# Jutho/KrylovKit.jl

Measured on NVIDIA H100. Metric: eigsolve_lanczos_operator_applications_per_sec, higher is better.
Workload: dtype f64

## Files before the change

krylovkit.jl_b200/csrc/basis.cu:

```cuda
#include "tsk.cuh"
#include <cmath>
#include <algorithm>

int32_t b2k_enqueue_dot(b2k_ctx* ctx, const void* q, void* x, int64_t n, const void* qprev,
                        int sprev_slot, int slot, int accum_slot);
int32_t b2k_enqueue_axpy_dev(b2k_ctx* ctx, void* x, const void* q, int s_slot, int64_t n);
int32_t b2k_enqueue_apply(b2k_ctx* ctx, const b2k_op* op, const VecRef& x, const VecRef& y,
                          double a0, double a1, bool shifted, const VecRef* dotv, int dot_slot);

using namespace tsk;

namespace {


template <typename T, bool UPDATE, bool PROJECT>
__global__ void __launch_bounds__(NTHREADS, 1)
k_phase(const __grid_constant__ PhaseParams<T> p, const __grid_constant__ ColList cl) {
    extern __shared__ __align__(128) uint8_t smem[];
    SmemView sm(smem);
    const int64_t ntiles = (p.n + Cfg<T>::R - 1) / Cfg<T>::R;
    const bool ragged = (p.n % Cfg<T>::R) != 0 && ((ntiles - 1) % gridDim.x) == blockIdx.x;
    pipe_setup(sm, ragged);
    Pipe st;
    if (threadIdx.x >= NCONS) producer_phase<T>(p, cl, sm, st);
    else consumer_phase<T, UPDATE, PROJECT>(p, sm, st);
}

template <typename T>
struct FusedParams {
    PhaseParams<T> ph[3];
    int32_t kind[3];
    int32_t nph;
    unsigned* barrier;
    unsigned barrier_base;
    const int* stop;
    FinalizeParams fin;
    PeerStep ps;
    unsigned long long* trace;
};

template <typename T>
__device__ __forceinline__ void peer_boundary(const FusedParams<T>& fp, int i, uint8_t* smem) {
    __threadfence();
    asm volatile("fence.proxy.async;" ::: "memory");
    __syncthreads();
    int* flag = reinterpret_cast<int*>(smem + OFF_RED + 256);
    if (threadIdx.x == 0) {
        const unsigned old = atomicAdd(fp.barrier, 1u);
        *flag = (old == fp.barrier_base + (unsigned)(i + 1) * gridDim.x - 1u);
    }
    __syncthreads();
    const PeerDev& pd = fp.ps.pd;
    const int tid = threadIdx.x;
    if (fp.ph[i].part_h == nullptr) {
        const unsigned long long sq = fp.ps.seq_norm;
        if (*flag && tid < 32) {
            __threadfence();
            double a = (tid < 16) ? partial_lane_sum(fp.ph[i].part_n, gridDim.x, 1, tid, 16) : 0.0;
            for (int o = 8; o > 0; o >>= 1) a += __shfl_xor_sync(0xffffffffu, a, o);
            if (tid == 0) peer_publish1(pd, PEER_CH_NORM, sq, a);
        }
        peer_wait(pd, PEER_CH_NORM, sq, tid);
        __syncthreads();
        return;
    }
    const unsigned long long seq = fp.ps.seq_coef[i];
    if (*flag && tid < NCONS) {
        __threadfence();
        const int k = fp.ph[i].k;
        const int L = coef_lanes(k);
        const int j = tid / L, l = tid % L;
        const bool valid = j < k;
        const double a = coef_colsum(fp.ph[i].part_h, gridDim.x, B2K_KSTRIDE, j, l, L, valid);
        if (valid && l == 0)
            for (int p = 0; p < pd.nranks; ++p) peer_slot(pd, p, PEER_CH_COEF, seq, pd.rank)[j] = a;
        __threadfence_system();
        named_bar_sync(1, NCONS);
        if (tid < pd.nranks) st_release_sys_u64(peer_flag(pd, tid, PEER_CH_COEF, seq, pd.rank), seq);
    }
    peer_wait(pd, PEER_CH_COEF, seq, tid);
    __syncthreads();
}

template <typename T>
__global__ void __launch_bounds__(NTHREADS, 1)
k_gs_fused(const __grid_constant__ FusedParams<T> fp, const __grid_constant__ ColList cl) {
    extern __shared__ __align__(128) uint8_t smem[];
    if (fp.stop && *reinterpret_cast<const volatile int*>(fp.stop)) {
        if (threadIdx.x == 0 && fp.nph > 1) atomicAdd(fp.barrier, (unsigned)(fp.nph - 1));
        return;
    }
    SmemView sm(smem);
    const bool tr0 = fp.trace && blockIdx.x == 0 && threadIdx.x == 0;
    if (tr0) b2k_trace(fp.trace, 10);
    const int64_t n = fp.ph[0].n;
    const int64_t ntiles = (n + Cfg<T>::R - 1) / Cfg<T>::R;
    const bool ragged = (n % Cfg<T>::R) != 0 && ((ntiles - 1) % gridDim.x) == blockIdx.x;
    pipe_setup(sm, ragged);
    Pipe st;
    const bool prod = threadIdx.x >= NCONS;
    if (fp.ps.on && fp.ps.seq_alpha && !prod) {
        peer_wait(fp.ps.pd, PEER_CH_ALPHA, fp.ps.seq_alpha, threadIdx.x);
        named_bar_sync(1, NCONS);
    }
    if (tr0) b2k_trace(fp.trace, 11);
    for (int i = 0; i < fp.nph; ++i) {
        if (prod) {
            producer_phase<T>(fp.ph[i], cl, sm, st);
        } else {
            if (fp.kind[i] == 0) consumer_phase<T, false, true>(fp.ph[i], sm, st);
            else if (fp.kind[i] == 1) consumer_phase<T, true, true>(fp.ph[i], sm, st);
            else consumer_phase<T, true, false>(fp.ph[i], sm, st);
        }
        if (tr0) b2k_trace(fp.trace, 12 + i);
        if (i + 1 < fp.nph) {
            if (fp.ps.on) peer_boundary<T>(fp, i, smem);
            else grid_barrier(fp.barrier, fp.barrier_base + (unsigned)(i + 1) * gridDim.x);
            if (tr0) b2k_trace(fp.trace, 15 + i);
        }
    }
    if (fp.fin.enabled && !prod) {
        double* sh = reinterpret_cast<double*>(smem + OFF_RED);
        int* flag = reinterpret_cast<int*>(smem + OFF_RED + 256);
        if (fp.ps.on) __threadfence_system();
        else __threadfence();
        named_bar_sync(1, NCONS);
        if (threadIdx.x == 0) {
            const unsigned t = atomicInc(fp.fin.ticket, gridDim.x - 1);
            *flag = (t == gridDim.x - 1);
        }
        named_bar_sync(1, NCONS);
        if (*flag) {
            __threadfence();
            if (fp.trace && threadIdx.x == 0) b2k_trace(fp.trace, 18);
            finalize_block(fp.fin, threadIdx.x, sh, fp.ps.on ? &fp.ps : nullptr);
            if (fp.trace && threadIdx.x == 0) b2k_trace(fp.trace, 19);
        }
    }
}

__global__ void __launch_bounds__(NCONS)
k_finalize(const double* __restrict__ A, const double* __restrict__ B, const double* __restrict__ N, int G,
           int stride, int k, double* __restrict__ res, int off, int noff) {
    __shared__ double sh[2];
    FinalizeParams f;
    f.A = A; f.B = B; f.N = N; f.G = G; f.stride = stride; f.k = k; f.res = res; f.off = off; f.noff = noff;
    f.rec = nullptr; f.alpha_col = -1; f.tol = 0.0; f.stop = nullptr; f.ticket = nullptr; f.enabled = 1;
    f.peer = 0; f.G_local = G; f.norm_done = 0;
    finalize_block(f, threadIdx.x, sh);
}

__global__ void k_lanczos_seed(double* rec, double beta, int* stop) {
    rec[2] = beta;
    rec[3] = 1.0 / beta;
    rec[4] = beta * beta;
    *stop = 0;
}

template <typename T>
__global__ void k_res_to_vec(const double* __restrict__ res, T* __restrict__ out, int k,
                             T alpha) {
    const int j = blockIdx.x * blockDim.x + threadIdx.x;
    if (j < k) out[j] = alpha * (T)res[j];
}

struct TransformParams {
    void* base;
    int64_t ld, n;
    int32_t m, keep, ldu;
    const double* U;
    int32_t u_in_smem;
};

constexpr int TR_OFF_U = NS * SLOT_BYTES;
constexpr int TR_U_BYTES = 232448 - TR_OFF_U - 256;
constexpr int TR_OFF_BAR = TR_OFF_U + TR_U_BYTES;
constexpr int TR_SMEM = TR_OFF_BAR + 2 * NS * 8;
constexpr int TJ = 36;
constexpr int TR_THREADS = NCONS + 32;

template <typename T, bool USM>
__global__ void __launch_bounds__(TR_THREADS, 1)
k_transform(const __grid_constant__ TransformParams p, const __grid_constant__ ColList cl) {
    using CF = Cfg<T>;
    using V16 = typename CF::V16;
    constexpr int R = CF::R, C = CF::C, VEC = CF::VEC;
    extern __shared__ __align__(128) uint8_t smem[];
    const uint32_t ring = smem_u32(smem);
    const uint32_t full = smem_u32(smem + TR_OFF_BAR), empty = full + NS * 8;
    T* Us = reinterpret_cast<T*>(smem + TR_OFF_U);
    const int pitch = ((p.keep + VEC - 1) / VEC) * VEC;
    if (threadIdx.x == 0) {
        for (int i = 0; i < NS; ++i) {
            mbar_init(full + 8 * i, 1);
            mbar_init(empty + 8 * i, NCONS / 32);
        }
        fence_mbar_init();
// ... 1391 lines not shown
    }

    B2K_TRY(b2k_enqueue_apply(ctx, op, rv, rw, 0.0, 1.0, false, nullptr, -1));
    B2K_TRY(b2k_vec_axpby(ctx, w, cols[k - 1], -beta_old, 1.0));
    B2K_TRY(b2k_enqueue_dot(ctx, rv.ptr, rw.ptr, pn.n, nullptr, -1, S_A0, -1));
    B2K_TRY(b2k_allreduce(ctx, ctx->d_res + S_A0, 1, pn.sharded));
    B2K_TRY(b2k_enqueue_axpy_dev(ctx, rw.ptr, rv.ptr, S_A0, pn.n));
    double alpha = 0.0, beta = 0.0;
    if (alg == B2K_MGS) {
        B2K_TRY(b2k_enqueue_dot(ctx, nullptr, rw.ptr, pn.n, nullptr, -1, S_N, -1));
        B2K_TRY(b2k_allreduce(ctx, ctx->d_res + S_N, 1, pn.sharded));
        B2K_TRY(b2k_fetch_results(ctx, S_A0 + 1, 0));
        alpha = ctx->h_res[S_A0];
        beta = sqrt(ctx->h_res[S_N]);
    } else if (alg == B2K_MGS2B) {
        if (fused_ok(ctx, K1, pn.sharded, ctx->dtype)) {
            if (f64) B2K_TRY(cgs_fused_t<double>(ctx, pn, rw, K1, 1, g_use_coop));
            else B2K_TRY(cgs_fused_t<float>(ctx, pn, rw, K1, 1, g_use_coop));
        } else {
            if (f64) B2K_TRY(cgs_pass_unfused_t<double>(ctx, pn, rw, K1, S_H, S_N));
            else B2K_TRY(cgs_pass_unfused_t<float>(ctx, pn, rw, K1, S_H, S_N));
        }
        B2K_TRY(b2k_fetch_results(ctx, S_A0 + 1, 0));
        alpha = ctx->h_res[S_A0] + ctx->h_res[S_H + k];
        beta = sqrt(ctx->h_res[S_N]);
    } else if (alg == B2K_MGS2) {
        B2K_TRY(mgs_sweep(ctx, pn, rw, K1, S_H, -1));
        B2K_TRY(b2k_enqueue_dot(ctx, nullptr, rw.ptr, pn.n, nullptr, -1, S_N, -1));
        B2K_TRY(b2k_allreduce(ctx, ctx->d_res + S_N, 1, pn.sharded));
        B2K_TRY(b2k_fetch_results(ctx, S_A0 + 1, 0));
        alpha = ctx->h_res[S_A0] + ctx->h_res[S_H + k];
        beta = sqrt(ctx->h_res[S_N]);
    } else {
        B2K_TRY(b2k_enqueue_dot(ctx, nullptr, rw.ptr, pn.n, nullptr, -1, S_N, -1));
        B2K_TRY(b2k_allreduce(ctx, ctx->d_res + S_N, 1, pn.sharded));
        B2K_TRY(b2k_fetch_results(ctx, S_A0 + 1, 0));
        alpha = ctx->h_res[S_A0];
        beta = sqrt(ctx->h_res[S_N]);
        double nold = sqrt(beta * beta + alpha * alpha + beta_old * beta_old);
        while (eps < beta && beta < eta * nold) {
            nold = beta;
            B2K_TRY(mgs_sweep(ctx, pn, rw, K1, S_H, -1));
            B2K_TRY(b2k_enqueue_dot(ctx, nullptr, rw.ptr, pn.n, nullptr, -1, S_N, -1));
            B2K_TRY(b2k_allreduce(ctx, ctx->d_res + S_N, 1, pn.sharded));
            B2K_TRY(b2k_fetch_results(ctx, S_N + 1, 0));
            alpha += ctx->h_res[S_H + k];
            beta = sqrt(ctx->h_res[S_N]);
        }
    }
    *alpha_out = alpha;
    *beta_out = beta;
    return B2K_OK;
}

bool g_use_chain = true;

bool chain_ok(const b2k_ctx* ctx, const b2k_op* op, const b2k_vec* cols, int32_t k, int32_t nsteps, int32_t alg,
              double beta_old) {
    if (!g_use_chain || !g_use_coop || (alg != B2K_CGS2 && alg != B2K_MGS2B) || nsteps < 1 || nsteps > B2K_MAX_CHAIN)
        return false;
    int64_t op_rows = 0, op_cols = 0;
    int32_t op_kind = -1;
    if (b2k_op_info(op, &op_rows, &op_cols, nullptr, &op_kind) != B2K_OK) return false;
    if ((op_kind != 0 && op_kind != 2) || beta_old == 0.0 || !(beta_old == beta_old)) return false;
    const int32_t sp = B2K_VEC_SPACE(cols[k]);
    if (sp < 0 || sp >= (int32_t)ctx->spaces.size()) return false;
    const B2kSpace& s = ctx->spaces[sp];
    if (ctx->nranks > 1) {
        if (!s.sharded || !b2k_peer_ok(ctx) || !b2k_op_has_peer_halo(op) || op_rows != s.n) return false;
    } else if (op_rows != s.n || op_cols != s.n) {
        return false;
    }
    const int C = ctx->dtype == B2K_F64 ? 8 : 16;
    const int K1 = k + nsteps;
    return (K1 + C - 1) / C <= NS && K1 <= MAXCH * C && K1 <= PEER_SLOT;
}

template <typename T>
int32_t chain_step_gs(b2k_ctx* ctx, const Panel& pn, int K1, const VecRef& rw, const VecRef& vprev,
                      const VecRef& rv, double* rec_prev, double* rec, double tol, const PeerStep* psp,
                      bool scale_after) {
    const int grid = grid_for_rows<T>(ctx, pn.n);
    ColList cl;
    for (int i = 0; i < K1; ++i) cl.c[i] = pn.idx[i];
    double* PA = b2k_part_set(ctx, 0);
    double* PN = b2k_part_set(ctx, 2);
    FusedParams<T> fp;
    memset(&fp, 0, sizeof(fp));
    PhaseParams<T> a = base_params<T>(pn, K1, rw.ptr, rw.ptr);
    a.nvec = 3; a.e1 = (const T*)vprev.ptr; a.e2 = (const T*)rv.ptr; a.store_x = 1;
    a.c1_dev = rec_prev + 2;
    a.c2_dev = rec + 0;
    a.part_h = PA;
    PhaseParams<T> c = base_params<T>(pn, K1, rw.ptr, rw.ptr);
    c.store_x = 1; c.coef = PA; c.coef_sets = grid; c.coef_stride = B2K_KSTRIDE;
    c.alphac = (T)-1; c.part_n = PN;
    fp.ph[0] = a; fp.kind[0] = 0; fp.ph[1] = c; fp.kind[1] = 2; fp.nph = 2;
    if (scale_after) {
        PhaseParams<T> sc = base_params<T>(pn, 0, rw.ptr, rw.ptr);
        sc.store_x = 1; sc.beta_mode = 2; sc.scale_mode = 1;
        sc.scale_norm = PN; sc.scale_G = grid; sc.scale_stride = 1; sc.scale_tol = tol;
        fp.ph[2] = sc; fp.kind[2] = 2; fp.nph = 3;
    }
    fp.stop = reinterpret_cast<const int*>(ctx->d_sync + B2K_SYNC_STOP);
    fp.trace = ctx->d_trace;
    fp.fin.A = PA; fp.fin.B = nullptr; fp.fin.N = PN; fp.fin.G = grid; fp.fin.stride = B2K_KSTRIDE;
    fp.fin.k = K1; fp.fin.res = nullptr; fp.fin.off = 0; fp.fin.noff = 0; fp.fin.rec = rec;
    fp.fin.alpha_col = K1 - 1; fp.fin.tol = tol;
    fp.fin.stop = reinterpret_cast<int*>(ctx->d_sync + B2K_SYNC_STOP);
    fp.fin.ticket = ctx->d_sync + B2K_SYNC_GSFIN; fp.fin.enabled = 1;
    fp.fin.peer = 0; fp.fin.G_local = grid; fp.fin.norm_done = 0;
    if (psp && psp->on) {
        const PeerStep& ps = *psp;
        fp.ps = ps;
        char* win = b2k_peer_local(ctx);
        auto slot = [&](int ch, unsigned long long seq) {
            return reinterpret_cast<double*>(win + PEER_OFF_SLOTS) + (size_t)((ch * 2 + (int)(seq & 1ull)) * PEER_MAXR) * PEER_SLOT;
        };
        fp.ph[0].c2_dev = slot(PEER_CH_ALPHA, ps.seq_alpha);
        fp.ph[0].c2_sets = ps.pd.nranks;
        fp.ph[0].c2_stride = PEER_SLOT;
        fp.ph[1].coef = slot(PEER_CH_COEF, ps.seq_coef[0]);
        fp.ph[1].coef_sets = ps.pd.nranks;
        fp.ph[1].coef_stride = PEER_SLOT;
        fp.fin.A = fp.ph[1].coef; fp.fin.G = ps.pd.nranks; fp.fin.stride = PEER_SLOT; fp.fin.peer = 1;
        const int last = fp.nph - 1;
        if (scale_after) {
            fp.ph[2].scale_norm = slot(PEER_CH_NORM, ps.seq_norm);
            fp.ph[2].scale_G = ps.pd.nranks;
            fp.ph[2].scale_stride = PEER_SLOT;
            fp.fin.norm_done = 1;
        }
        if (ps.seq_halo) {
            fp.ph[last].send_lo = ps.send_lo;
            fp.ph[last].send_hi = ps.send_hi;
            fp.ph[last].halo_dn = ps.send_lo ? reinterpret_cast<T*>(ps.pd.win[ps.pd.rank - 1] + ps.dn_off) : nullptr;
            fp.ph[last].halo_up = ps.send_hi ? reinterpret_cast<T*>(ps.pd.win[ps.pd.rank + 1] + ps.up_off) : nullptr;
        }
    }
    const int pr = b2k_prof_begin(ctx, 1, (2.0 * K1 + 3.0) * sizeof(T) * (double)pn.n);
    B2K_TRY(launch_fused<T>(ctx, fp, cl, grid));
    b2k_prof_end(ctx, pr);
    return B2K_OK;
}

int32_t lanczos_chain(b2k_ctx* ctx, const b2k_op* op, b2k_vec* cols, int32_t k, int32_t nsteps,
                      double beta_old, double tol, int32_t alg, double* alphas_out, double* betas_out,
                      int32_t* steps_done, b2k_vec* r_out) {
    const bool f64 = ctx->dtype == B2K_F64;
    const int32_t space = B2K_VEC_SPACE(cols[k]);
    double* rec0 = ctx->d_steps;
    int* d_stop = reinterpret_cast<int*>(ctx->d_sync + B2K_SYNC_STOP);
    {
        VecRef t;
        for (int i = 0; i <= k; ++i) B2K_TRY(b2k_resolve(ctx, cols[i], &t));
    }
    k_lanczos_seed<<<1, 1, 0, ctx->stream>>>(rec0, beta_old, d_stop);
    B2K_LAUNCH_CHECK(ctx);
    const bool inplace = g_chain_mode == 1;
    std::vector<b2k_vec> touched, Vh, Wh;
    touched.push_back(cols[k]);
    int32_t enq = 0, rc = B2K_OK;
    const bool dist = ctx->nranks > 1;
    unsigned long long halo_seq = 0;
    if (inplace) B2K_TRY(b2k_vec_scale(ctx, cols[k], cols[k], 1.0 / beta_old));
    for (int32_t i = 0; i < nsteps; ++i) {
        const int32_t K = k + i;
        const b2k_vec R = cols[K];
        b2k_vec V = R, W = -1;
        if (!inplace) {
            rc = b2k_vec_alloc(ctx, space, &V);
            if (rc != B2K_OK) break;
            touched.push_back(V);
        }
        rc = b2k_vec_alloc(ctx, space, &W);
        if (rc != B2K_OK) break;
        touched.push_back(W);
        VecRef rR, rV, rW, vprev;
        rc = b2k_resolve(ctx, R, &rR);
        if (rc == B2K_OK) rc = b2k_resolve(ctx, V, &rV);
        if (rc == B2K_OK) rc = b2k_resolve(ctx, W, &rW);
        if (rc == B2K_OK) rc = b2k_resolve(ctx, cols[K - 1], &vprev);
        if (rc != B2K_OK) break;
        double* rec_prev = rec0 + (size_t)B2K_REC * i;
        double* rec = rec0 + (size_t)B2K_REC * (i + 1);
        const bool scale_after = inplace && (i + 1 < nsteps);
        SpmvFuse fz;
        memset(&fz, 0, sizeof(fz));
        if (!inplace) {
            fz.xscale = rec_prev + 3;
            fz.vout = rV.ptr;
        }
        fz.stop = d_stop;
        fz.dot_self = 1;
        fz.l2_hints = g_l2_hints ? 1 : 0;
        fz.trace = ctx->d_trace;
        if (alg == B2K_MGS2B) {
            fz.dot_sub_vec = vprev.ptr;
            fz.dot_sub_scale = rec_prev + 2;
        }
        PeerStep ps;
        memset(&ps, 0, sizeof(ps));
        if (dist) {
            ps.on = 1;
// ... 186 lines not shown
        CoefList cf;
        for (int i = 0; i < kk; ++i) {
            cl.c[i] = pn.idx[off + i];
            cf.c[i] = alpha * x_host[off + i];
        }
        const int bm = beta == 1.0 ? 1 : (beta == 0.0 ? 0 : 2);
        if (ctx->dtype == B2K_F64)
            k_rank1<double><<<grid, 256, 0, ctx->stream>>>((double*)pn.base, pn.ld, pn.n, kk,
                                                           (const double*)ry.ptr, beta, bm, cl, cf);
        else
            k_rank1<float><<<grid, 256, 0, ctx->stream>>>((float*)pn.base, pn.ld, pn.n, kk,
                                                          (const float*)ry.ptr, (float)beta, bm, cl, cf);
        B2K_LAUNCH_CHECK(ctx);
    }
    return B2K_OK;
}

extern "C" int32_t b2k_basis_householder(b2k_ctx* ctx, const b2k_vec* cols, int32_t k,
                                         const double* v_host, double beta, b2k_vec work) {
    if (!ctx) return B2K_EINVAL;
    if (beta == 0.0 || k == 0) return B2K_OK;
    B2K_TRY(b2k_basis_unproject(ctx, work, cols, k, v_host, 1.0, 0.0));
    return b2k_basis_rank1update(ctx, cols, k, work, v_host, -beta, 1.0);
}



extern "C" int32_t b2k_block_reorthogonalize(b2k_ctx* ctx, const b2k_vec* Rb, int32_t p,
                                             const b2k_vec* V, int32_t k) {
    if (!ctx || !Rb || p < 1) return B2K_EINVAL;
    if (k == 0) return B2K_OK;
    Panel pn;
    B2K_TRY(make_panel(ctx, V, k, &pn));
    if (k > B2K_RES_DOUBLES - 8) return b2k_fail(ctx, B2K_ENOTSUP, "block_reorthogonalize: k too large");
    for (int i = 0; i < p; ++i) {
        VecRef rv;
        B2K_TRY(b2k_resolve(ctx, Rb[i], &rv));
        if (rv.n != pn.n) return b2k_fail(ctx, B2K_EDIM, "block_reorthogonalize: length mismatch");
        B2K_TRY(mgs_sweep(ctx, pn, rv, k, 0, -1));
    }
    return B2K_OK;
}

extern "C" int32_t b2k_block_qr(b2k_ctx* ctx, const b2k_vec* X, int32_t p, double tol,
                                double* R_host, int32_t* good, int32_t* drift) {
    if (!ctx || !X || !R_host || !good || !drift || p < 1) return B2K_EINVAL;
    for (int i = 0; i < p * p; ++i) R_host[i] = 0.0;
    *drift = 0;
    double nrm;
    B2K_TRY(b2k_vec_norm(ctx, X[0], &nrm));
    if (nrm > tol) {
        R_host[0] = nrm;
        B2K_TRY(b2k_vec_scale(ctx, X[0], X[0], 1.0 / nrm));
        good[0] = 1;
    } else {
        B2K_TRY(b2k_vec_zero(ctx, X[0]));
        good[0] = 0;
    }
    std::vector<double> h(p);
    for (int j = 1; j < p; ++j) {
        double beta;
        int32_t passes;
        B2K_TRY(b2k_basis_orthogonalize(ctx, X[j], X, j, h.data(), B2K_MGS, 0.0, &beta, &passes));
        for (int i = 0; i < j; ++i) R_host[(size_t)j * p + i] = h[i];
        if (tol < beta && beta < 100 * tol) {
            *drift = 1;
            B2K_TRY(b2k_basis_orthogonalize(ctx, X[j], X, j, h.data(), B2K_MGS, 0.0, &beta, &passes));
            for (int i = 0; i < j; ++i) R_host[(size_t)j * p + i] += h[i];
        }
        if (beta < tol) {
            B2K_TRY(b2k_vec_zero(ctx, X[j]));
            good[j] = 0;
        } else {
            R_host[(size_t)j * p + j] = beta;
            B2K_TRY(b2k_vec_scale(ctx, X[j], X[j], 1.0 / beta));
            good[j] = 1;
        }
    }
    return B2K_OK;
}

extern "C" int32_t b2k_debug_trace(b2k_ctx* ctx, int32_t on) {
    if (!ctx) return B2K_EINVAL;
    if (on) {
        if (!ctx->d_trace) B2K_CUDA(ctx, cudaMalloc(&ctx->d_trace, sizeof(unsigned long long) * (2 + 2 * B2K_TRACE_CAP)));
        B2K_CUDA(ctx, cudaMemsetAsync(ctx->d_trace, 0, sizeof(unsigned long long) * 2, ctx->stream));
    } else if (ctx->d_trace) {
        B2K_TRY(b2k_stream_sync(ctx));
        cudaFree(ctx->d_trace);
        ctx->d_trace = nullptr;
    }
    return B2K_OK;
}

extern "C" int32_t b2k_debug_trace_read(b2k_ctx* ctx, unsigned long long* out, int64_t cap_events, int64_t* n_events) {
    if (!ctx || !out || !n_events) return B2K_EINVAL;
    *n_events = 0;
    if (!ctx->d_trace) return B2K_OK;
    B2K_TRY(b2k_stream_sync(ctx));
    unsigned long long cnt = 0;
    B2K_CUDA(ctx, cudaMemcpy(&cnt, ctx->d_trace, sizeof(cnt), cudaMemcpyDeviceToHost));
    if (cnt > B2K_TRACE_CAP) cnt = B2K_TRACE_CAP;
    if ((int64_t)cnt > cap_events) cnt = (unsigned long long)cap_events;
    B2K_CUDA(ctx, cudaMemcpy(out, ctx->d_trace + 2, sizeof(unsigned long long) * 2 * cnt, cudaMemcpyDeviceToHost));
    *n_events = (int64_t)cnt;
    return B2K_OK;
}
```

krylovkit.jl_b200/csrc/common.cuh:

```cuda
#pragma once
#include <cuda_runtime.h>
#include <cstdint>
#include <cstdio>
#include <cstring>
#include <string>
#include <vector>
#include "../../include/b200krylov.h"

constexpr int B2K_MAX_SPACES   = 8;
constexpr int B2K_RES_DOUBLES  = 8192;
constexpr int B2K_COEF_DOUBLES = 65536;
constexpr int B2K_MAX_GRID     = 1024;
constexpr int B2K_KSTRIDE      = 256;
constexpr int B2K_MAX_CHAIN    = 512;
constexpr int B2K_REC          = 8;
constexpr int B2K_SYNC_GSFIN   = 2;
constexpr int B2K_SYNC_STOP    = 4;
constexpr int B2K_SYNC_HALO    = 5;

struct B2kSpace {
    void*   base   = nullptr;
    int64_t n      = 0;
    int64_t ld     = 0;
    int32_t ncols  = 0;
    int32_t sharded = 1;
    std::vector<uint8_t> used;
};

struct B2kNccl;

constexpr int B2K_PROF_CLASSES = 9;
struct B2kProfRec { int cls; double bytes; cudaEvent_t e0, e1; };
struct B2kProf {
    bool on = false;
    std::vector<cudaEvent_t> pool;
    size_t next = 0;
    std::vector<B2kProfRec> recs;
};

struct b2k_ctx {
    int32_t device = 0;
    int32_t dtype  = B2K_F64;
    int32_t esize  = 8;
    int32_t num_sms = 0;
    size_t  l2_persist_bytes = 0;
    int     dot_hints = 0;
    unsigned long long* d_trace = nullptr;
    size_t  l2_window_max = 0;
    cudaStream_t stream = nullptr;
    std::vector<B2kSpace> spaces;
    std::vector<b2k_op*> ops;

    double*   d_part   = nullptr;
    double*   d_part_s = nullptr;
    double*   d_res    = nullptr;
    double*   h_res    = nullptr;
    double*   d_coef   = nullptr;
    double*   h_coef   = nullptr;
    unsigned* d_sync   = nullptr;
    double*   d_steps  = nullptr;
    double*   d_blk    = nullptr;
    double*   d_blkpart = nullptr;
    cudaEvent_t ev_coef = nullptr;
    cudaEvent_t ev_t0 = nullptr, ev_t1 = nullptr;
    bool      coef_busy = false;

    int32_t rank = 0, nranks = 1;
    int64_t n_global = 0, row_offset = 0;
    B2kNccl* nccl = nullptr;

    B2kProf prof;
    unsigned barrier_base = 0;
    int64_t launches = 0;
    std::string err;
};

extern std::string g_b2k_create_error;

int32_t b2k_fail(b2k_ctx* ctx, int32_t code, const char* fmt, ...);

#define B2K_CUDA(ctx, call)                                                              \
    do {                                                                                 \
        cudaError_t e__ = (call);                                                        \
        if (e__ != cudaSuccess)                                                          \
            return b2k_fail((ctx), B2K_ECUDA, "%s:%d: %s -> %s", __FILE__, __LINE__,     \
                            #call, cudaGetErrorString(e__));                             \
    } while (0)

#define B2K_TRY(call)                                                                    \
    do {                                                                                 \
        int32_t s__ = (call);                                                            \
        if (s__ != B2K_OK) return s__;                                                   \
    } while (0)

#define B2K_LAUNCH_CHECK(ctx)                                                            \
    do {                                                                                 \
        (ctx)->launches++;                                                               \
        cudaError_t e__ = cudaGetLastError();                                            \
        if (e__ != cudaSuccess)                                                          \
            return b2k_fail((ctx), B2K_ECUDA, "%s:%d: kernel launch -> %s", __FILE__,    \
                            __LINE__, cudaGetErrorString(e__));                          \
    } while (0)

struct VecRef {
    void*   ptr;
    int64_t n;
    int64_t ld;
    int32_t space;
    int32_t col;
    int32_t sharded;
};

int32_t b2k_resolve(b2k_ctx* ctx, b2k_vec v, VecRef* out);
int32_t b2k_resolve_cols(b2k_ctx* ctx, const b2k_vec* cols, int32_t k, int32_t* space,
                         std::vector<int32_t>* idx);

int32_t b2k_fetch_results(b2k_ctx* ctx, int32_t count, int32_t sharded);
int32_t b2k_allreduce(b2k_ctx* ctx, double* dptr, int32_t count, int32_t sharded);
int32_t b2k_put_coef(b2k_ctx* ctx, const double* host, int32_t count, int32_t offset);

cudaError_t b2k_dmalloc(void** p, size_t bytes, cudaStream_t stream);
cudaError_t b2k_dfree(void* p, cudaStream_t stream);
#define B2K_DMALLOC(p, bytes) b2k_dmalloc((void**)(p), (bytes), ctx->stream)
#define B2K_DFREE(p) b2k_dfree((p), ctx->stream)
cudaError_t b2k_hmalloc(void** p, size_t bytes);
void b2k_hfree(void* p, size_t bytes);

int  b2k_prof_begin(b2k_ctx* ctx, int cls, double bytes);
void b2k_prof_end(b2k_ctx* ctx, int idx);

// ... 252 lines not shown
```

krylovkit.jl_b200/csrc/tsk.cuh:

```cuda
#pragma once
#include "common.cuh"

namespace tsk {

template <typename T> struct Cfg;
template <> struct Cfg<double> {
    static constexpr int R = 256, C = 8, VEC = 2;
    using V16 = double2;
    __device__ static __forceinline__ void unpack(const double2& v, double* o) { o[0] = v.x; o[1] = v.y; }
};
template <> struct Cfg<float> {
    static constexpr int R = 256, C = 16, VEC = 4;
    using V16 = float4;
    __device__ static __forceinline__ void unpack(const float4& v, float* o) {
        o[0] = v.x; o[1] = v.y; o[2] = v.z; o[3] = v.w;
    }
};

constexpr int NS = 12;
constexpr int NW = 3;
constexpr int NCONS = 256;
constexpr int NPROD = 4;
constexpr int NTHREADS = NCONS + 32 * NPROD;
constexpr int MAXCH = 16;
constexpr int SLOT_BYTES = 16384;
static_assert(NS % NPROD == 0, "a ring slot must always be refilled by the same producer warp");

template <typename T> constexpr int kcap() { return MAXCH * Cfg<T>::C; }

constexpr int OFF_RING = 0;
constexpr int OFF_WRING = NS * SLOT_BYTES;
constexpr int WSLOT_MAX = 3 * 256 * 8;
constexpr int OFF_W1 = OFF_WRING + NW * WSLOT_MAX;
constexpr int OFF_CS = OFF_W1 + 2 * 256 * 8;
constexpr int OFF_RED = OFF_CS + 1024;
constexpr int OFF_BAR = OFF_RED + 512;
constexpr int SMEM_BYTES = OFF_BAR + (2 * NS + 2 * NW) * 8;

struct ColList {
    int32_t c[256];
};

template <typename T>
struct PhaseParams {
    const T* base;
    int64_t ld;
    int64_t n;
    int32_t k;
    const T* x;
    T* xout;
    const T* e1;
    const T* e2;
    T c1, c2;
    const double* c1_dev;
    const double* c2_dev;
    int32_t c2_sets;
    int32_t c2_stride;
    T* halo_dn;
    T* halo_up;
    int64_t send_lo, send_hi;
    int32_t scale_mode;
    const double* scale_norm;
    int32_t scale_G, scale_stride;
    double scale_tol;
    int32_t nvec;
    int32_t store_x;
    int32_t l2_hints;
    const double* coef;
    const T* coef_t;
    int32_t coef_sets;
    int32_t coef_stride;
    T alphac, betax;
    int32_t beta_mode;
    double* part_h;
    double* part_n;
};

struct Pipe {
    uint32_t s = 0, ph = 0, ws = 0, wph = 0;
    uint32_t g = 0;
};

struct SmemView {
    uint8_t* raw;
    uint32_t ring, wring, full, empty, wfull, wempty;
    __device__ explicit SmemView(uint8_t* p) : raw(p) {
        ring = smem_u32(p + OFF_RING);
        wring = smem_u32(p + OFF_WRING);
        full = smem_u32(p + OFF_BAR);
        empty = full + NS * 8;
        wfull = empty + NS * 8;
        wempty = wfull + NW * 8;
    }
};

__device__ __forceinline__ void pipe_setup(const SmemView& sm, bool zero_ring) {
    if (threadIdx.x == 0) {
        for (int i = 0; i < NS; ++i) {
            mbar_init(sm.full + 8 * i, 1);
            mbar_init(sm.empty + 8 * i, NCONS / 32);
        }
        for (int i = 0; i < NW; ++i) {
            mbar_init(sm.wfull + 8 * i, 1);
            mbar_init(sm.wempty + 8 * i, NCONS / 32);
        }
        fence_mbar_init();
    }
    if (zero_ring) {
        uint4* q = reinterpret_cast<uint4*>(sm.raw);
        for (int i = threadIdx.x; i < OFF_CS / 16; i += blockDim.x) q[i] = make_uint4(0, 0, 0, 0);
        fence_proxy_async();
    }
    __syncthreads();
}

__device__ __forceinline__ int coef_lanes(int k) {
    int L = 16;
    while (L > 1 && L * k > NCONS) L >>= 1;
    return L;
}
__device__ __forceinline__ double partial_lane_sum(const double* P, int G, int stride, int l, int L) {
    double a = 0.0;
    int g = l;
    for (; g + 11 * L < G; g += 12 * L) {
        double t[12];
#pragma unroll
        for (int u = 0; u < 12; ++u) t[u] = __ldcg(P + (size_t)(g + u * L) * stride);
#pragma unroll
        for (int u = 0; u < 12; ++u) a += t[u];
    }
    for (; g + 3 * L < G; g += 4 * L) {
        const double t0 = __ldcg(P + (size_t)g * stride), t1 = __ldcg(P + (size_t)(g + L) * stride);
        const double t2 = __ldcg(P + (size_t)(g + 2 * L) * stride), t3 = __ldcg(P + (size_t)(g + 3 * L) * stride);
        a += t0; a += t1; a += t2; a += t3;
    }
    for (; g < G; g += L) a += __ldcg(P + (size_t)g * stride);
    return a;
}
__device__ __forceinline__ double coef_colsum(const double* P, int G, int stride, int j, int l, int L,
                                              bool valid) {
    double a = valid ? partial_lane_sum(P + j, G, stride, l, L) : 0.0;
    for (int o = L >> 1; o > 0; o >>= 1) a += __shfl_xor_sync(0xffffffffu, a, o);
    return a;
}

template <typename T>
__device__ __forceinline__ void producer_phase(const PhaseParams<T>& p, const ColList& cl,
                                               const SmemView& sm, Pipe& st) {
    using CF = Cfg<T>;
    constexpr int R = CF::R, C = CF::C;
    const int lane = threadIdx.x & 31;
    const uint32_t me = (threadIdx.x - NCONS) >> 5;
    const int nch = (p.k + C - 1) / C;
    const int64_t ntiles = (p.n + R - 1) / R;
    const uint64_t pol = p.l2_hints ? l2_policy_evict_first() : 0;
    for (int64_t tile = blockIdx.x; tile < ntiles; tile += gridDim.x) {
        const int64_t r0 = tile * R;
        const int rt = (int)((p.n - r0) < R ? (p.n - r0) : R);
        const uint32_t bytes = (uint32_t)((rt * sizeof(T) + 15) & ~(size_t)15);
        if (me == 0) {
            mbar_wait(sm.wempty + 8 * st.ws, st.wph ^ 1);
            if (lane == 0) mbar_expect_tx(sm.wfull + 8 * st.ws, bytes * (uint32_t)p.nvec);
            __syncwarp();
            if (lane < p.nvec) {
                const T* src = (lane == 0) ? p.x : (lane == 1 ? p.e1 : p.e2);
                bulk_g2s(sm.wring + st.ws * (3 * R * (int)sizeof(T)) + lane * R * (int)sizeof(T),
                         src + r0, bytes, sm.wfull + 8 * st.ws);
            }
        }
        if (++st.ws == NW) { st.ws = 0; st.wph ^= 1; }
        for (int c = 0; c < nch; ++c) {
            if ((st.g % NPROD) == me) {
                mbar_wait(sm.empty + 8 * st.s, st.ph ^ 1);
                const int ncol = (p.k - c * C) < C ? (p.k - c * C) : C;
                if (lane == 0) mbar_expect_tx(sm.full + 8 * st.s, bytes * (uint32_t)ncol);
                __syncwarp();
                if (lane < ncol) {
                    const T* src = p.base + (int64_t)cl.c[c * C + lane] * p.ld + r0;
                    if (p.l2_hints)
                        bulk_g2s_hint(sm.ring + st.s * SLOT_BYTES + lane * R * (int)sizeof(T), src, bytes,
                                      sm.full + 8 * st.s, pol);
                    else
                        bulk_g2s(sm.ring + st.s * SLOT_BYTES + lane * R * (int)sizeof(T), src, bytes,
                                 sm.full + 8 * st.s);
                }
            }
            ++st.g;
            if (++st.s == NS) { st.s = 0; st.ph ^= 1; }
        }
    }
}

template <typename T> struct VecOps;
template <> struct VecOps<double> {
    __device__ static __forceinline__ void fma_acc(double& acc, const double2& q, const double2& x) {
        acc = fma(q.x, x.x, acc);
        acc = fma(q.y, x.y, acc);
    }
};
template <> struct VecOps<float> {
    __device__ static __forceinline__ void fma_acc(float& acc, const float4& q, const float4& x) {
        acc = fmaf(q.x, x.x, acc);
        acc = fmaf(q.y, x.y, acc);
        acc = fmaf(q.z, x.z, acc);
        acc = fmaf(q.w, x.w, acc);
    }
};

template <typename T, bool UPDATE, bool PROJECT>
__device__ __forceinline__ void consumer_phase(const PhaseParams<T>& p, const SmemView& sm,
                                               Pipe& st) {
    using CF = Cfg<T>;
    using V16 = typename CF::V16;
    constexpr int R = CF::R, C = CF::C, VEC = CF::VEC;
    constexpr int CPW = C / 8;
    constexpr int NLD = R / (32 * VEC);
    const int tid = threadIdx.x;
    const int lane = tid & 31, w = tid >> 5;
    const int nch = (p.k + C - 1) / C;
    const int64_t ntiles = (p.n + R - 1) / R;
    T* cs = reinterpret_cast<T*>(sm.raw + OFF_CS);
    T* w1 = reinterpret_cast<T*>(sm.raw + OFF_W1);
    double* red = reinterpret_cast<double*>(sm.raw + OFF_RED);

    if (UPDATE) {
        if (p.coef_t) {
            for (int j = tid; j < p.k; j += NCONS) cs[j] = p.alphac * p.coef_t[j];
        } else {
            const int L = coef_lanes(p.k);
            const int j = tid / L, l = tid % L;
            const bool valid = j < p.k;
            const double h = coef_colsum(p.coef, p.coef_sets, p.coef_stride, j, l, L, valid);
            if (valid && l == 0) cs[j] = p.alphac * (T)h;
        }
        named_bar_sync(1, NCONS);
    }

    T acc_h[MAXCH][CPW];
#pragma unroll
    for (int c = 0; c < MAXCH; ++c)
#pragma unroll
        for (int cc = 0; cc < CPW; ++cc) acc_h[c][cc] = (T)0;
    T nrm = (T)0;
    int buf = 0;
    const uint64_t pol_last = p.l2_hints ? l2_policy_evict_last() : 0;
    T betax = p.betax;
    bool do_store = p.store_x != 0;
    if (UPDATE && p.scale_mode) {
        double* shn = reinterpret_cast<double*>(sm.raw + OFF_RED + 128);
        if (tid < 32) {
            double a;
            if (p.scale_stride == 1) {
                a = (tid < 16) ? partial_lane_sum(p.scale_norm, p.scale_G, 1, tid, 16) : 0.0;
                for (int o = 8; o > 0; o >>= 1) a += __shfl_xor_sync(0xffffffffu, a, o);
            } else {
                a = 0.0;
                for (int g = 0; g < p.scale_G; ++g)
                    a += *reinterpret_cast<const volatile double*>(p.scale_norm + (size_t)g * p.scale_stride);
            }
            if (tid == 0) shn[0] = a;
        }
        named_bar_sync(1, NCONS);
        const double beta = sqrt(shn[0]);
        if (beta <= p.scale_tol) do_store = false;
        betax = (T)(1.0 / beta);
    }
    T c1 = p.c1, c2 = p.c2;
    if (p.c1_dev) c1 = (T)(-(*reinterpret_cast<const volatile double*>(p.c1_dev)));
    if (p.c2_dev) {
        double a2 = 0.0;
        const int ns = p.c2_sets > 1 ? p.c2_sets : 1;
        for (int g = 0; g < ns; ++g)
            a2 += *reinterpret_cast<const volatile double*>(p.c2_dev + (size_t)g * p.c2_stride);
        c2 = (T)(-a2);
    }

    for (int64_t tile = blockIdx.x; tile < ntiles; tile += gridDim.x) {
        const int64_t r0 = tile * R;
        const int rt = (int)((p.n - r0) < R ? (p.n - r0) : R);
        mbar_wait(sm.wfull + 8 * st.ws, st.wph);
        const T* wv = reinterpret_cast<const T*>(sm.raw + OFF_WRING) + st.ws * 3 * R;
        T xv = wv[tid];
        if (p.nvec == 3) {
            xv = fma(c1, wv[R + tid], xv);
            xv = fma(c2, wv[2 * R + tid], xv);
        }
        if (tid >= rt) xv = (T)0;
        T acc = xv;
        const uint32_t s0 = st.s, ph0 = st.ph;
        if (UPDATE) {
            acc = (p.beta_mode == 0) ? (T)0 : (p.beta_mode == 1 ? xv : betax * xv);
            for (int c = 0; c < nch; ++c) {
                mbar_wait(sm.full + 8 * st.s, st.ph);
                const T* slot = reinterpret_cast<const T*>(sm.raw + OFF_RING + st.s * SLOT_BYTES);
                const int ncol = (p.k - c * C) < C ? (p.k - c * C) : C;
                if (ncol == C) {
                    T cv[C];
#pragma unroll
                    for (int i = 0; i < C / VEC; ++i)
                        CF::unpack(*reinterpret_cast<const V16*>(cs + c * C + i * VEC), cv + i * VEC);
#pragma unroll
                    for (int jj = 0; jj < C; ++jj) acc = fma(slot[jj * R + tid], cv[jj], acc);
                } else {
                    for (int jj = 0; jj < ncol; ++jj) acc = fma(slot[jj * R + tid], cs[c * C + jj], acc);
                }
                if (!PROJECT) {
                    __syncwarp();
                    if (lane == 0) mbar_arrive(sm.empty + 8 * st.s);
                }
                if (++st.s == NS) { st.s = 0; st.ph ^= 1; }
            }
            if (tid >= rt) acc = (T)0;
        }
        if (do_store && tid < rt) {
            if (p.l2_hints) st_hint(p.xout + r0 + tid, acc, pol_last);
            else p.xout[r0 + tid] = acc;
            if (UPDATE && !PROJECT) {
                const int64_t r = r0 + tid;
                if (p.halo_dn && r < p.send_lo) p.halo_dn[r] = acc;
                if (p.halo_up && r >= p.n - p.send_hi) p.halo_up[r - (p.n - p.send_hi)] = acc;
            }
        }
        if (p.part_n) nrm = fma(acc, acc, nrm);
        if (PROJECT) {
            T* wb = w1 + buf * R;
            wb[tid] = acc;
            named_bar_sync(1, NCONS);
            V16 xr[NLD];
#pragma unroll
            for (int i = 0; i < NLD; ++i)
                xr[i] = *reinterpret_cast<const V16*>(wb + VEC * lane + 32 * VEC * i);
            uint32_t ss = UPDATE ? s0 : st.s, pp = UPDATE ? ph0 : st.ph;
#pragma unroll
            for (int c = 0; c < MAXCH; ++c) {
                if (c < nch) {
                    if (!UPDATE) mbar_wait(sm.full + 8 * ss, pp);
                    const T* slot = reinterpret_cast<const T*>(sm.raw + OFF_RING + ss * SLOT_BYTES);
#pragma unroll
                    for (int cc = 0; cc < CPW; ++cc) {
                        const int cj = cc * 8 + w;
                        if (c * C + cj < p.k) {
                            const T* colp = slot + cj * R;
#pragma unroll
                            for (int i = 0; i < NLD; ++i) {
                                V16 q = *reinterpret_cast<const V16*>(colp + VEC * lane + 32 * VEC * i);
                                VecOps<T>::fma_acc(acc_h[c][cc], q, xr[i]);
                            }
                        }
                    }
                    __syncwarp();
                    if (lane == 0) mbar_arrive(sm.empty + 8 * ss);
                    if (++ss == NS) { ss = 0; pp ^= 1; }
                }
            }
            if (!UPDATE) { st.s = ss; st.ph = pp; }
            buf ^= 1;
        }
        __syncwarp();
        if (lane == 0) mbar_arrive(sm.wempty + 8 * st.ws);
        if (++st.ws == NW) { st.ws = 0; st.wph ^= 1; }
    }

    if (PROJECT) {
#pragma unroll
        for (int c = 0; c < MAXCH; ++c) {
#pragma unroll
            for (int cc = 0; cc < CPW; ++cc) {
                const int j = c * C + cc * 8 + w;
                double v = warp_sum((double)acc_h[c][cc]);
                if (c < nch && j < p.k && lane == 0)
                    p.part_h[(size_t)blockIdx.x * B2K_KSTRIDE + j] = v;
            }
        }
    }
    if (p.part_n) {
        double v = warp_sum((double)nrm);
        if (lane == 0) red[w] = v;
        named_bar_sync(1, NCONS);
        if (tid == 0) {
            double s = 0.0;
#pragma unroll
            for (int i = 0; i < NCONS / 32; ++i) s += red[i];
            p.part_n[blockIdx.x] = s;
        }
    }
}

struct FinalizeParams {
    const double* A;
    const double* B;
    const double* N;
    int G, stride, k;
    double* res;
    int off, noff;
    double* rec;
    int alpha_col;
    double tol;
    int* stop;
    unsigned* ticket;
    int enabled;
    int peer;
    int G_local;
    int norm_done;
};

__device__ __forceinline__ void finalize_block(const FinalizeParams& f, int tid, double* sh,
                                               const PeerStep* ps = nullptr) {
    double hval = 0.0;
    if (f.k > 0) {
        const int L = coef_lanes(f.k);
        const int j = tid / L, l = tid % L;
        const bool valid = j < f.k;
        double a = coef_colsum(f.A, f.G, f.stride, j, l, L, valid);
        if (f.B) a += coef_colsum(f.B, f.G, f.stride, j, l, L, valid);
        if (valid && l == 0) {
            if (f.res) f.res[f.off + j] = a;
            if (j == f.alpha_col) hval = a;
        }
        if (f.rec && valid && l == 0 && j == f.alpha_col) sh[0] = hval;
    }
    double n2 = 0.0;
    if (f.N && tid < 32) {
        double a = (tid < 16) ? partial_lane_sum(f.N, f.peer ? f.G_local : f.G, 1, tid, 16) : 0.0;
        for (int o = 8; o > 0; o >>= 1) a += __shfl_xor_sync(0xffffffffu, a, o);
        n2 = a;
    }
    double alpha0 = f.rec ? f.rec[0] : 0.0;
    if (f.peer && ps) {
        if (!f.norm_done) {
            if (tid == 0) peer_publish1(ps->pd, PEER_CH_NORM, ps->seq_norm, n2);
            peer_wait(ps->pd, PEER_CH_NORM, ps->seq_norm, tid);
        }
        named_bar_sync(1, NCONS);
        if (tid == 0) {
            n2 = peer_sum1(ps->pd, PEER_CH_NORM, ps->seq_norm, 0);
            if (ps->seq_alpha) alpha0 = peer_sum1(ps->pd, PEER_CH_ALPHA, ps->seq_alpha, 0);
            if (ps->seq_halo) {
                __threadfence_system();
                if (ps->send_lo) st_relaxed_sys_u64(peer_hflag(ps->pd, ps->pd.rank - 1, ps->seq_halo, 1), ps->seq_halo);
                if (ps->send_hi) st_relaxed_sys_u64(peer_hflag(ps->pd, ps->pd.rank + 1, ps->seq_halo, 0), ps->seq_halo);
            }
        }
    }
    if (f.N && tid == 0 && f.res) f.res[f.noff] = n2;
    if (f.rec) {
        named_bar_sync(1, NCONS);
        if (tid == 0) {
            f.rec[0] = alpha0;
            const double alpha = alpha0 + sh[0];
            const double beta = sqrt(n2);
            f.rec[1] = alpha;
            f.rec[2] = beta;
            f.rec[3] = 1.0 / beta;
            f.rec[4] = n2;
// ... 20 lines not shown
```

Before: 335.3.

## Read last two Lanczos vectors from basis ring instead of separate streams

Reorders the column list so the two most recent basis vectors come first in the panel ring, and the three-term recurrence reads them from the ring slot instead of loading vprev and rv as extra streamed vectors. Phase one no longer stores x, and phase two recomputes the recurrence from the ring. Coefficient and partial-sum indices are permuted to match. The aim is to cut global memory traffic per Lanczos step, at the cost of more index bookkeeping and extra FMAs. It also adds an optional per-CTA trace hook.

```diff
diff --git a/krylovkit.jl_b200/csrc/basis.cu b/krylovkit.jl_b200/csrc/basis.cu
--- a/krylovkit.jl_b200/csrc/basis.cu
+++ b/krylovkit.jl_b200/csrc/basis.cu
@@ -37,6 +37,7 @@
     FinalizeParams fin;
     PeerStep ps;
     unsigned long long* trace;
+    unsigned long long* trace_ctas;
 };
 
 template <typename T>
@@ -113,6 +114,7 @@
             else consumer_phase<T, true, false>(fp.ph[i], sm, st);
         }
         if (tr0) b2k_trace(fp.trace, 12 + i);
+        if (fp.trace_ctas && threadIdx.x == 0) b2k_trace(fp.trace_ctas, (blockIdx.x << 8) | (20u + (unsigned)i));
         if (i + 1 < fp.nph) {
             if (fp.ps.on) peer_boundary<T>(fp, i, smem);
             else grid_barrier(fp.barrier, fp.barrier_base + (unsigned)(i + 1) * gridDim.x);
@@ -1670,17 +1672,20 @@
                       bool scale_after) {
     const int grid = grid_for_rows<T>(ctx, pn.n);
     ColList cl;
-    for (int i = 0; i < K1; ++i) cl.c[i] = pn.idx[i];
+    cl.c[0] = pn.idx[K1 - 2];
+    cl.c[1] = pn.idx[K1 - 1];
+    for (int i = 0; i + 2 < K1; ++i) cl.c[i + 2] = pn.idx[i];
     double* PA = b2k_part_set(ctx, 0);
     double* PN = b2k_part_set(ctx, 2);
     FusedParams<T> fp;
     memset(&fp, 0, sizeof(fp));
-    PhaseParams<T> a = base_params<T>(pn, K1, rw.ptr, rw.ptr);
-    a.nvec = 3; a.e1 = (const T*)vprev.ptr; a.e2 = (const T*)rv.ptr; a.store_x = 1;
+    PhaseParams<T> a = base_params<T>(pn, K1, rw.ptr, nullptr);
+    a.lead2 = 1;
     a.c1_dev = rec_prev + 2;
     a.c2_dev = rec + 0;
     a.part_h = PA;
     PhaseParams<T> c = base_params<T>(pn, K1, rw.ptr, rw.ptr);
+    c.lead2 = 1; c.c1_dev = a.c1_dev; c.c2_dev = a.c2_dev;
     c.store_x = 1; c.coef = PA; c.coef_sets = grid; c.coef_stride = B2K_KSTRIDE;
     c.alphac = (T)-1; c.part_n = PN;
     fp.ph[0] = a; fp.kind[0] = 0; fp.ph[1] = c; fp.kind[1] = 2; fp.nph = 2;
@@ -1692,6 +1697,7 @@
     }
     fp.stop = reinterpret_cast<const int*>(ctx->d_sync + B2K_SYNC_STOP);
     fp.trace = ctx->d_trace;
+    fp.trace_ctas = ctx->trace_ctas ? ctx->d_trace : nullptr;
     fp.fin.A = PA; fp.fin.B = nullptr; fp.fin.N = PN; fp.fin.G = grid; fp.fin.stride = B2K_KSTRIDE;
     fp.fin.k = K1; fp.fin.res = nullptr; fp.fin.off = 0; fp.fin.noff = 0; fp.fin.rec = rec;
     fp.fin.alpha_col = K1 - 1; fp.fin.tol = tol;
@@ -1705,9 +1711,11 @@
         auto slot = [&](int ch, unsigned long long seq) {
             return reinterpret_cast<double*>(win + PEER_OFF_SLOTS) + (size_t)((ch * 2 + (int)(seq & 1ull)) * PEER_MAXR) * PEER_SLOT;
         };
-        fp.ph[0].c2_dev = slot(PEER_CH_ALPHA, ps.seq_alpha);
-        fp.ph[0].c2_sets = ps.pd.nranks;
-        fp.ph[0].c2_stride = PEER_SLOT;
+        for (int i = 0; i < 2; ++i) {
+            fp.ph[i].c2_dev = slot(PEER_CH_ALPHA, ps.seq_alpha);
+            fp.ph[i].c2_sets = ps.pd.nranks;
+            fp.ph[i].c2_stride = PEER_SLOT;
+        }
         fp.ph[1].coef = slot(PEER_CH_COEF, ps.seq_coef[0]);
         fp.ph[1].coef_sets = ps.pd.nranks;
         fp.ph[1].coef_stride = PEER_SLOT;
@@ -2060,6 +2068,7 @@
 
 extern "C" int32_t b2k_debug_trace(b2k_ctx* ctx, int32_t on) {
     if (!ctx) return B2K_EINVAL;
+    ctx->trace_ctas = on == 2;
     if (on) {
         if (!ctx->d_trace) B2K_CUDA(ctx, cudaMalloc(&ctx->d_trace, sizeof(unsigned long long) * (2 + 2 * B2K_TRACE_CAP)));
         B2K_CUDA(ctx, cudaMemsetAsync(ctx->d_trace, 0, sizeof(unsigned long long) * 2, ctx->stream));
diff --git a/krylovkit.jl_b200/csrc/common.cuh b/krylovkit.jl_b200/csrc/common.cuh
--- a/krylovkit.jl_b200/csrc/common.cuh
+++ b/krylovkit.jl_b200/csrc/common.cuh
@@ -46,6 +46,7 @@
     size_t  l2_persist_bytes = 0;
     int     dot_hints = 0;
     unsigned long long* d_trace = nullptr;
+    bool    trace_ctas = false;
     size_t  l2_window_max = 0;
     cudaStream_t stream = nullptr;
     std::vector<B2kSpace> spaces;
diff --git a/krylovkit.jl_b200/csrc/tsk.cuh b/krylovkit.jl_b200/csrc/tsk.cuh
--- a/krylovkit.jl_b200/csrc/tsk.cuh
+++ b/krylovkit.jl_b200/csrc/tsk.cuh
@@ -64,6 +64,7 @@
     int32_t scale_G, scale_stride;
     double scale_tol;
     int32_t nvec;
+    int32_t lead2;
     int32_t store_x;
     int32_t l2_hints;
     const double* coef;
@@ -223,15 +224,16 @@
     T* w1 = reinterpret_cast<T*>(sm.raw + OFF_W1);
     double* red = reinterpret_cast<double*>(sm.raw + OFF_RED);
 
+    auto pos = [&](int j) { return !p.lead2 ? j : (j >= p.k - 2 ? j - (p.k - 2) : j + 2); };
     if (UPDATE) {
         if (p.coef_t) {
-            for (int j = tid; j < p.k; j += NCONS) cs[j] = p.alphac * p.coef_t[j];
+            for (int j = tid; j < p.k; j += NCONS) cs[pos(j)] = p.alphac * p.coef_t[j];
         } else {
             const int L = coef_lanes(p.k);
             const int j = tid / L, l = tid % L;
             const bool valid = j < p.k;
             const double h = coef_colsum(p.coef, p.coef_sets, p.coef_stride, j, l, L, valid);
-            if (valid && l == 0) cs[j] = p.alphac * (T)h;
+            if (valid && l == 0) cs[pos(j)] = p.alphac * (T)h;
         }
         named_bar_sync(1, NCONS);
     }
@@ -285,6 +287,15 @@
             xv = fma(c1, wv[R + tid], xv);
             xv = fma(c2, wv[2 * R + tid], xv);
         }
+        T e1v = (T)0, e2v = (T)0;
+        if (p.lead2) {
+            mbar_wait(sm.full + 8 * st.s, st.ph);
+            const T* slot = reinterpret_cast<const T*>(sm.raw + OFF_RING + st.s * SLOT_BYTES);
+            e1v = slot[tid];
+            e2v = slot[R + tid];
+            xv = fma(c1, e1v, xv);
+            xv = fma(c2, e2v, xv);
+        }
         if (tid >= rt) xv = (T)0;
         T acc = xv;
         const uint32_t s0 = st.s, ph0 = st.ph;
@@ -294,21 +305,27 @@
                 mbar_wait(sm.full + 8 * st.s, st.ph);
                 const T* slot = reinterpret_cast<const T*>(sm.raw + OFF_RING + st.s * SLOT_BYTES);
                 const int ncol = (p.k - c * C) < C ? (p.k - c * C) : C;
+                const int j0 = (p.lead2 && c == 0) ? 2 : 0;
                 if (ncol == C) {
                     T cv[C];
 #pragma unroll
                     for (int i = 0; i < C / VEC; ++i)
                         CF::unpack(*reinterpret_cast<const V16*>(cs + c * C + i * VEC), cv + i * VEC);
 #pragma unroll
-                    for (int jj = 0; jj < C; ++jj) acc = fma(slot[jj * R + tid], cv[jj], acc);
+                    for (int jj = 0; jj < C; ++jj)
+                        if (jj >= j0) acc = fma(slot[jj * R + tid], cv[jj], acc);
                 } else {
-                    for (int jj = 0; jj < ncol; ++jj) acc = fma(slot[jj * R + tid], cs[c * C + jj], acc);
+                    for (int jj = j0; jj < ncol; ++jj) acc = fma(slot[jj * R + tid], cs[c * C + jj], acc);
                 }
                 if (!PROJECT) {
                     __syncwarp();
                     if (lane == 0) mbar_arrive(sm.empty + 8 * st.s);
                 }
                 if (++st.s == NS) { st.s = 0; st.ph ^= 1; }
+            }
+            if (p.lead2) {
+                acc = fma(e1v, cs[0], acc);
+                acc = fma(e2v, cs[1], acc);
             }
             if (tid >= rt) acc = (T)0;
         }
@@ -368,8 +385,10 @@
             for (int cc = 0; cc < CPW; ++cc) {
                 const int j = c * C + cc * 8 + w;
                 double v = warp_sum((double)acc_h[c][cc]);
-                if (c < nch && j < p.k && lane == 0)
-                    p.part_h[(size_t)blockIdx.x * B2K_KSTRIDE + j] = v;
+                if (c < nch && j < p.k && lane == 0) {
+                    const int jo = !p.lead2 ? j : (j < 2 ? p.k - 2 + j : j - 2);
+                    p.part_h[(size_t)blockIdx.x * B2K_KSTRIDE + jo] = v;
+                }
             }
         }
     }
```

Result: faster. 343.3, median of 6 (+2.4%).
